# permon/permon

Measured on AMD Instinct MI355X. Metric: QPS iterations/sec + CSR SpMV GB/s (% HBM roofline), higher is better.
Workload: dtype f64; 1 GPU; configs[2]: 3-D elasticity TFETI contact, 2x2x2 subdomains of 43^3 Q1 elements (N=2044416 dof, n_lambda=102268), SMALXE+MPGP on the dual QP, F = B K^+ B' with K^+ explicit (dense local dual operators, storage class_orbit)

## Files before the change

### include/permon_hip.h

```cpp
#ifndef PERMON_HIP_H
#define PERMON_HIP_H

#include <stddef.h>
#include <stdint.h>

#ifdef __cplusplus
extern "C" {
#endif

#define PMH_SUCCESS 0
#define PMH_ERR_HIP 1
#define PMH_ERR_ARG 2
#define PMH_ERR_STATE 3
#define PMH_ERR_SUP 4
#define PMH_ERR_NODEVICE 5
#define PMH_ERR_COMM 6
const char *pmh_last_error(void);

#define PMH_CONVERGED_ITERATING 0
#define PMH_CONVERGED_RTOL 2
#define PMH_CONVERGED_ATOL 3
#define PMH_CONVERGED_ITS 4
#define PMH_CONVERGED_HAPPY_BREAKDOWN 7
#define PMH_DIVERGED_ITS (-3)
// ... 589 lines not shown
  double        astol, afeas, alpha, acg_host, pAp_host;
  double        ttol, divtol_rhs, gamma2;
  double        ring[48];
  double        scal_dev[64], scal_pinned[64];
  int           emit;
  int           spec;
  int           setp;
  int           finalize;
  int           use_ctl;
  int           nb;
  int           ring_cap, max_it;
  int           ctl[4];
} pmh_mpgp_phase_test;
enum { PMH_PHASE_SPLIT = 0, PMH_PHASE_STEP, PMH_PHASE_DIR, PMH_PHASE_PROP_DIR, PMH_PHASE_EXPANSION, PMH_PHASE_P1_DOTS, PMH_PHASE_THREE_NORMS, PMH_PHASE_OBJ };
int pmh_vec_test_finalize(pmh_ctx ctx, int K, int nblocks, const double *rows_host, const int *ops, const int *slots, int halt, int *post_inc, double *scal_dev, double *scal_pinned);
int pmh_mpgp_test_host_sum_row(const double *row, int nb, int op, double *out);
int pmh_mpgp_test_block_sum(pmh_ctx ctx, int nb, const double *row_host, double *out_host);
int pmh_mpgp_test_block_partials(pmh_ctx ctx, int n, const double *a, const double *b, const double *c, double *dev_host, double *pinned_host);
int pmh_mpgp_test_phase(pmh_ctx ctx, int phase, int n, pmh_mpgp_phase_test *t);
int pmh_mpgp_test_set_gradient_valid(pmh_mpgp s, const double *g);
int pmh_mpgp_test_spec_words(pmh_mpgp s, int words[5]);
int pmh_op_test_create_staged(pmh_csr gather, pmh_csr middle, pmh_csr scatter, pmh_op *op);
int pmh_op_penalized_test_chain_info(pmh_op op, long long info[10]);
int pmh_op_penalized_test_chain_read(pmh_op op, int what, int cap, double *host, int *len);
int pmh_op_penalized_test_norm_target(pmh_op op, double *Gu, int slot, const double *u, int *ready);
int pmh_op_penalized_test_mult_epi2(pmh_op op, int kind, int same_input, int in_slot, const double *x, const double *b, const double *g, const double *xx, const double *lb,
                                    const double *ub, double astol, double *y, double *gf, double *p, double *partials_dev_host, double *partials_pinned_host, int *nblocks,
                                    int *replayed);
int pmh_op_penalized_test_form(pmh_op op, int *form);
int pmh_op_penalized_test_aux_normG(pmh_op op, int armed, const double *u, double *Gu, int slot, const double *x, double *y, double scal[2], int *served);
// ... 17 lines not shown
```

### permon_amd/_lib.py

```python
import ctypes as C
import os

_HERE = os.path.dirname(os.path.abspath(__file__))
LIB_PATH = os.path.join(_HERE, "libpermonhip.so")

c_double_p = C.POINTER(C.c_double)
c_int_p = C.POINTER(C.c_int)
vp = C.c_void_p


class PermonHipError(RuntimeError):
    pass


class MpgpOpts(C.Structure):
    _fields_ = [
        ("rtol", C.c_double), ("atol", C.c_double), ("divtol", C.c_double), ("max_it", C.c_int),
        ("alpha_user", C.c_double), ("alpha_direct", C.c_int), ("gamma", C.c_double),
        ("maxeig", C.c_double), ("maxeig_tol", C.c_double), ("maxeig_iter", C.c_int),
        ("bchop_tol", C.c_double), ("astol", C.c_double),
        ("exptype", C.c_int), ("explengthtype", C.c_int),
        ("resetalpha", C.c_int), ("fallback", C.c_int), ("fallback2", C.c_int),
        ("monitor", C.c_int), ("unfused", C.c_int), ("distributed", C.c_int),
    ]
# ... 370 lines not shown
    "pmh_mg_create_sa": [vp, vp, C.c_int, vp, C.c_int, vp, vp, vp, C.c_int, vp, C.c_int, vp, C.c_int, C.c_double, C.c_int, C.c_int, C.POINTER(vp)],
    "pmh_mg_timing_enable": [vp, C.c_int],
    "pmh_mg_timing_get": [vp, C.POINTER(C.c_int), C.POINTER(C.c_double), C.POINTER(C.c_double)],
    "pmh_matinv_enable_bsr3": [vp],
    "pmh_matinv_bsr3_replicas": [vp, c_int_p],
    "pmh_mv_test_spmv": [vp, C.c_int, vp, vp, C.c_int, C.POINTER(C.c_float)],
    "pmh_mv_test_create": [vp, C.c_int, C.c_int, C.c_int, C.POINTER(vp)],
    "pmh_mv_test_info": [vp, C.POINTER(C.c_longlong), c_double_p],
    "pmh_mv_test_mult_epi": [vp, C.c_int, vp, vp, vp, vp, vp, vp, vp, C.c_double, C.c_double, C.c_double, C.c_int],
    "pmh_mv_test_destroy": [vp],
    "pmh_csr_kernel_info": [vp, c_int_p, C.POINTER(C.c_ulonglong)],
    "pmh_csr_test_mult_epi": [vp, C.c_int, vp, vp, vp, vp, vp, vp, C.c_int, vp, c_double_p],
    "pmh_op_penalized_test_mult_epi": [vp, C.c_int, C.c_int, vp, vp, vp, C.c_double, vp, vp, vp, C.c_int, vp, vp, c_int_p, c_int_p],
    "pmh_op_penalized_test_emit": [vp, C.c_int, vp],
    "pmh_vec_test_finalize": [vp, C.c_int, C.c_int, vp, vp, vp, C.c_int, vp, vp, vp],
    "pmh_mpgp_test_host_sum_row": [vp, C.c_int, C.c_int, c_double_p],
    "pmh_mpgp_test_block_sum": [vp, C.c_int, vp, vp],
    "pmh_mpgp_test_block_partials": [vp, C.c_int, vp, vp, vp, vp, vp],
    "pmh_mpgp_test_phase": [vp, C.c_int, C.c_int, C.POINTER(MpgpPhaseTest)],
    "pmh_mpgp_test_set_gradient_valid": [vp, vp],
    "pmh_mpgp_test_spec_words": [vp, c_int_p],
    "pmh_op_test_create_staged": [vp, vp, vp, C.POINTER(vp)],
    "pmh_op_penalized_test_chain_info": [vp, C.POINTER(C.c_longlong)],
    "pmh_op_penalized_test_chain_read": [vp, C.c_int, C.c_int, vp, c_int_p],
    "pmh_op_penalized_test_norm_target": [vp, vp, C.c_int, vp, c_int_p],
    "pmh_op_penalized_test_mult_epi2": [vp, C.c_int, C.c_int, C.c_int, vp, vp, vp, vp, vp, vp, C.c_double, vp, vp, vp, vp, vp, c_int_p, c_int_p],
    "pmh_op_penalized_test_form": [vp, c_int_p],
    "pmh_op_penalized_test_aux_normG": [vp, C.c_int, vp, vp, C.c_int, vp, vp, c_double_p, c_int_p],
    "pmh_bsr3_test_create": [vp, C.c_int, C.c_int, C.c_int, C.POINTER(vp)],
    "pmh_bsr3_test_info": [vp, C.POINTER(C.c_longlong), c_double_p],
# ... 106 lines not shown
```

### permon_amd/csrc/ctx.hip

```cpp
#include <sched.h>

#include <algorithm>
#include <thread>

#include "pmh_internal.h"

static thread_local char g_err[1024] = "";

int pmh_set_error(int code, const char *fmt, ...)
{
  va_list ap;
  va_start(ap, fmt);
  vsnprintf(g_err, sizeof(g_err), fmt, ap);
  va_end(ap);
  return code;
}

extern "C" const char *pmh_last_error(void) { return g_err; }

pmh_knobs_s &pmh_knobs()
{
  static pmh_knobs_s k = [] {
    pmh_knobs_s v;
    v.chain = getenv("PMH_NO_CHAIN") ? 0 : 1;
    v.chain_replay = getenv("PMH_NO_CHAIN_REPLAY") ? 0 : 1;
    v.svm_pairing = getenv("PMH_SVM_NO_PAIRING") ? 0 : 1;
    v.gt_fusion = getenv("PMH_NO_GT_FUSION") ? 0 : 1;
    v.multi_rhs = getenv("PMH_NO_MULTI_RHS") ? 0 : 1;
    v.kplus_mv = getenv("PMH_NO_KPLUS_MV") ? 0 : 1;
    v.smalxe_prefetch = getenv("PMH_SMALXE_NO_PREFETCH") ? 0 : 1;
    v.mg_d0_fusion = getenv("PMH_MG_NO_D0_FUSION") ? 0 : 1;
    v.vec_epi = getenv("PMH_NO_VEC_EPI") ? 0 : 1;
    v.mpgp_spec = getenv("PMH_MPGP_NO_SPEC") ? 0 : 1;
    v.orbit_adapted = getenv("PMH_NO_ORBIT_ADAPTED") ? 0 : 1;
    int         nt = 0;
    const char *e  = getenv("PMH_HOST_THREADS");
    if (!e) e = getenv("OMP_NUM_THREADS");
    if (e) nt = atoi(e);
    if (nt <= 0) {
      cpu_set_t set;
      CPU_ZERO(&set);
      nt = (sched_getaffinity(0, sizeof(set), &set) == 0) ? CPU_COUNT(&set) : (int)std::thread::hardware_concurrency();
      nt = std::min(16, nt);
    }
    v.host_threads = std::max(1, std::min(64, nt));
// ... 4 lines not shown
static int *knob_by_name(const char *name)
{
  if (!name) return nullptr;
  if (!strcmp(name, "chain")) return &pmh_knobs().chain;
  if (!strcmp(name, "chain_applies")) return &pmh_knobs().chain_applies;
  if (!strcmp(name, "chain_launches")) return &pmh_knobs().chain_launches;
  if (!strcmp(name, "chain_replay")) return &pmh_knobs().chain_replay;
  if (!strcmp(name, "chain_replays")) return &pmh_knobs().chain_replays;
  if (!strcmp(name, "chain_replays_redone")) return &pmh_knobs().chain_replays_redone;
  if (!strcmp(name, "host_threads")) return &pmh_knobs().host_threads;
  if (!strcmp(name, "svm_pairing")) return &pmh_knobs().svm_pairing;
  if (!strcmp(name, "gt_fusion")) return &pmh_knobs().gt_fusion;
  if (!strcmp(name, "multi_rhs")) return &pmh_knobs().multi_rhs;
  if (!strcmp(name, "kplus_mv")) return &pmh_knobs().kplus_mv;
  if (!strcmp(name, "smalxe_prefetch")) return &pmh_knobs().smalxe_prefetch;
  if (!strcmp(name, "mg_d0_fusion")) return &pmh_knobs().mg_d0_fusion;
  if (!strcmp(name, "mpgp_spec")) return &pmh_knobs().mpgp_spec;
  if (!strcmp(name, "vec_epi")) return &pmh_knobs().vec_epi;
  if (!strcmp(name, "orbit_adapted")) return &pmh_knobs().orbit_adapted;
  if (!strcmp(name, "orbit_adapted_classes")) return &pmh_knobs().orbit_adapted_classes;
  if (!strcmp(name, "orbit_adapted_fallbacks")) return &pmh_knobs().orbit_adapted_fallbacks;
  if (!strcmp(name, "orbit_adapted_spoil")) return &pmh_knobs().orbit_adapted_spoil;
  return nullptr;
}
extern "C" int pmh_set_knob(const char *name, int value)
{
  int *k = knob_by_name(name);
  if (!k) return pmh_set_error(PMH_ERR_ARG, "pmh_set_knob: unknown switch '%s'", name ? name : "(null)");
  *k = value;
  return PMH_SUCCESS;
// ... 67 lines not shown
  hipDeviceProp_t prop;
  PMH_HIP(hipGetDeviceProperties(&prop, c->device));
  snprintf(buf, len, "%s (%s, %d CUs)", prop.name, prop.gcnArchName, prop.multiProcessorCount);
  return PMH_SUCCESS;
}

extern "C" int pmh_mem_info(pmh_ctx c, size_t *free_bytes, size_t *total_bytes)
{
  PMH_ARG(c && free_bytes && total_bytes);
  PMH_HIP(hipSetDevice(c->device));
  PMH_HIP(hipStreamSynchronize(c->stream));
  PMH_HIP(hipMemGetInfo(free_bytes, total_bytes));
  return PMH_SUCCESS;
}

static inline hipError_t ctx_wait(pmh_ctx c) { return hipStreamSynchronize(c->stream); }

extern "C" int pmh_sync(pmh_ctx c)
{
  PMH_ARG(c);
  PMH_HIP(ctx_wait(c));
  return PMH_SUCCESS;
}

extern "C" void *pmh_stream(pmh_ctx c) { return c ? (void *)c->stream : nullptr; }

extern "C" int pmh_malloc(pmh_ctx c, size_t bytes, void **dptr)
{
  PMH_ARG(c && dptr);
  PMH_HIP(hipSetDevice(c->device));
  PMH_HIP(hipMalloc(dptr, bytes ? bytes : 8));
// ... 225 lines not shown
```

### permon_amd/csrc/dualchain.h

```cpp
#pragma once
#include "pmh_internal.h"

struct pmh_dualchain_s;
typedef pmh_dualchain_s *pmh_dualchain;

int  pmh_dc_create(pmh_qppf pf, pmh_op F, pmh_dualchain *out);
void pmh_dc_destroy(pmh_dualchain dc);
int  pmh_dc_apply(pmh_dualchain dc, const double *x, double *y, double rho, const pmh_vec_epi *epi);
int  pmh_dc_emit_begin(pmh_dualchain dc, const double *x, const double *p, pmh_emit_args *ea);
void pmh_dc_invalidate(pmh_dualchain dc, bool keep_applied = false);
int  pmh_dc_replay(pmh_dualchain dc, const double *x, double *y, double rho, const pmh_vec_epi *epi, int *replayed);
int  pmh_dc_test_emit(pmh_dualchain dc, const double *x);
int  pmh_dc_test_direction_sums(pmh_dualchain dc, int cap, double *host, int *nseg);
int  pmh_dc_set_norm_target(pmh_dualchain dc, double *Gu, int slot);
bool pmh_dc_norm_ready(pmh_dualchain dc, const double *u);
int  pmh_dc_last_launches(pmh_dualchain dc);
int  pmh_dc_test_info(pmh_dualchain dc, long long info[10]);
int  pmh_dc_test_read(pmh_dualchain dc, int what, int cap, double *host, int *len);
```

### permon_amd/csrc/dualchain.hip

```cpp
#include <algorithm>
#include <cmath>
#include <type_traits>

#include "dualchain.h"
#include "emit_inline.h"
#include "box_inline.h"
#include "reduce.h"

struct pmh_dualchain_s {
  pmh_ctx  ctx;
  pmh_qppf pf;
  pmh_op   F;
  int      n, m, nwg, nseg, W;
  pmh_csr  gather = nullptr, scatter = nullptr;
  double  *mid_in = nullptr;
  const double *mid_out = nullptr;
  int     *d_seg = nullptr, *d_lrow = nullptr;
  double        *d_ev = nullptr;
  unsigned char *d_ec = nullptr;
  pmh_csr  list_for = nullptr;
  unsigned long long list_uid = 0, sc_uid = 0;
  double  *zeroed   = nullptr;
  int      nlist = 0, *d_reci = nullptr;
  double  *d_recd = nullptr;
  pmh_csr  sc_for = nullptr;
  int     *d_sc2 = nullptr;
  double  *d_sv2 = nullptr;
  unsigned char *d_scnt = nullptr;
  double  *part[3] = {nullptr, nullptr, nullptr};
  double  *c_cur   = nullptr;
  double  *w       = nullptr;
  double  *normGu    = nullptr;
  int      norm_slot = -1;
  const double *x_emitted = nullptr;
  bool     norm_done = false;
  const double *norm_ptr = nullptr;
  int      launches = 0;
  const double      *kept_x     = nullptr;
  unsigned long long kept_epoch = 0;
};


__global__ __launch_bounds__(PMH_EMIT_TILE) void k_dc_emit(int n, const double *__restrict__ x, pmh_emit_args ea)
{
  pmh_emit_regs R;
  pmh_emit_prefetch(ea, R);
  const int r = blockIdx.x * PMH_EMIT_TILE + threadIdx.x;
  pmh_emit_tail(ea, R, r < n ? x[r] : 0.0, 0.0);
}

template <int NU>
// ... 449 lines not shown
}

static void dc_launch_emit(pmh_dualchain dc, const double *x, double *part)
{
  hipLaunchKernelGGL(k_dc_emit, dim3((unsigned)dc->nwg), dim3(PMH_EMIT_TILE), 0, dc->ctx->stream, dc->n, x, dc_emit_args(dc, part, nullptr));
}

int pmh_dc_emit_begin(pmh_dualchain dc, const double *x, const double *p, pmh_emit_args *ea)
{
  *ea = dc_emit_args(dc, x ? dc->part[0] : nullptr, p ? dc->part[1] : nullptr);
  if ((x && x == dc->kept_x) || (p && p == dc->kept_x)) dc->kept_x = nullptr;
  if (x) dc->x_emitted = x, dc->norm_done = false, dc->norm_ptr = nullptr;
  return PMH_SUCCESS;
}

void pmh_dc_invalidate(pmh_dualchain dc, bool keep_applied)
{
  dc->x_emitted = nullptr, dc->norm_ptr = nullptr, dc->norm_done = false;
  if (!keep_applied) dc->kept_x = nullptr;
}

int pmh_dc_set_norm_target(pmh_dualchain dc, double *Gu, int slot)
{
  PMH_ARG(dc && Gu && slot >= 0 && slot < PMH_NSCAL);
  dc->normGu = Gu, dc->norm_slot = slot, dc->norm_ptr = nullptr, dc->norm_done = false;
  return PMH_SUCCESS;
}

bool pmh_dc_norm_ready(pmh_dualchain dc, const double *u)
{
  if (!dc || !dc->normGu) return false;
  if (dc->norm_ptr == u) return true;
  if (dc->x_emitted == u && !dc->norm_done) {
// ... 34 lines not shown
  });
  dc->launches++;
  PMH_HIP(hipGetLastError());
  return PMH_SUCCESS;
}

int pmh_dc_apply(pmh_dualchain dc, const double *x, double *y, double rho, const pmh_vec_epi *epi)
{
  pmh_ctx     ctx = dc->ctx;
  hipStream_t st  = ctx->stream;
  const int   n = dc->n;
  const dim3  vgrid((unsigned)dc->nwg), eblk(PMH_EMIT_TILE);
  const int   kind = epi ? epi->kind : 0;
  dc->launches     = 0;
  dc->kept_x       = nullptr;
  const pmh_emit_tab tab = dc_tab(dc);
  int slot = (epi && epi->in_slot > 0) ? epi->in_slot - 1 : -1;
  if (slot < 0) {
    slot = (kind == PMH_VEPI_GRAD_SPLIT) ? 0 : (kind == PMH_VEPI_P1 ? 1 : 2);
    if (slot == 0) dc->x_emitted = x, dc->norm_done = false, dc->norm_ptr = nullptr;
    dc_launch_emit(dc, x, dc->part[slot]);
    dc->launches++;
  }
  PMH_CHK(dc->F->stages(&dc->gather, &dc->mid_in, &dc->scatter, &dc->mid_out));
  const pmh_csr Bg = dc->gather, Bs = dc->scatter;
  if (Bg->ncols != n || Bs->nrows != n) return pmh_set_error(PMH_ERR_STATE, "pmh_dc_apply: the operator's stages changed their dual dimension");
  PMH_CHK(dc_prepare_stages(dc));
  {
    dc_norm_args na;
    memset(&na, 0, sizeof(na));
// ... 25 lines not shown
int pmh_dc_replay(pmh_dualchain dc, const double *x, double *y, double rho, const pmh_vec_epi *epi, int *replayed)
{
  const int kind = epi ? epi->kind : 0;
  if (replayed) *replayed = 0;
  bool      ok   = pmh_knobs().chain_replay && x && dc->kept_x == x && dc->kept_epoch == dc->ctx->free_epoch && (kind == 0 || kind == PMH_VEPI_GRAD_SPLIT);
  if (ok) {
    pmh_csr       g = nullptr, sc = nullptr;
    double       *mi = nullptr;
    const double *mo = nullptr;
    PMH_CHK(dc->F->stages(&g, &mi, &sc, &mo));
    ok = g && sc && g == dc->list_for && g->uid == dc->list_uid && mi == dc->zeroed && sc == dc->sc_for && sc->uid == dc->sc_uid && mo == dc->mid_out;
  }
  if (!ok) return pmh_dc_apply(dc, x, y, rho, epi);
  dc->launches = 0;
  if (kind == PMH_VEPI_GRAD_SPLIT && !(epi->in_slot > 0)) {
    dc->x_emitted = x, dc->norm_done = false, dc->norm_ptr = nullptr;
    dc_launch_emit(dc, x, dc->part[0]);
    dc->launches++;
  }
  PMH_CHK(dc_last_stage(dc, x, y, rho, epi));
  if (replayed) *replayed = 1;
  pmh_knobs().chain_applies++, pmh_knobs().chain_replays++, pmh_knobs().chain_launches += dc->launches;
  return PMH_SUCCESS;
}

int pmh_dc_test_emit(pmh_dualchain dc, const double *x)
{
  pmh_emit_args ea;
  PMH_CHK(pmh_dc_emit_begin(dc, x, nullptr, &ea));
  dc_launch_emit(dc, x, ea.o[0].part);
  PMH_HIP(hipGetLastError());
  return PMH_SUCCESS;
}
int pmh_dc_test_direction_sums(pmh_dualchain dc, int cap, double *host, int *nseg)
// ... 81 lines not shown
```

### permon_amd/csrc/pmh_internal.h

```cpp
#pragma once
#include <hip/hip_runtime.h>
#include <rccl/rccl.h>

#include <cstdarg>
#include <cstdio>
#include <cstdlib>
#include <cstring>
#include <vector>

#include "permon_hip.h"

#define PMH_BLOCK 256
#define PMH_MAX_VEC_BLOCKS 2048
#define PMH_MAX_RED 8
#define PMH_NSCAL 64

int pmh_set_error(int code, const char *fmt, ...);

struct pmh_knobs_s {
  int chain;
  int chain_applies = 0, chain_launches = 0;
  int chain_replay = 1, chain_replays = 0, chain_replays_redone = 0;
  int gt_fusion = 1;
  int smalxe_prefetch = 1;
  int vec_epi = 1;
  int orbit_adapted = 1, orbit_adapted_classes = 0, orbit_adapted_fallbacks = 0, orbit_adapted_spoil = 0;
  int mpgp_spec = 1;
  int mg_d0_fusion = 1;
  int kplus_mv = 1;
  int multi_rhs = 1;
  int svm_pairing = 1;
  int host_threads = 1;
};
pmh_knobs_s &pmh_knobs();
inline int   pmh_host_threads() { return pmh_knobs().host_threads > 1 ? pmh_knobs().host_threads : 1; }

#define PMH_HIP(call) \
  do { \
    hipError_t e_ = (call); \
// ... 17 lines not shown
struct pmh_ctx_s {
  int         device;
  int         num_cus;
  hipStream_t stream;
  hipEvent_t  ev0, ev1;
  double     *d_partials;
  int         partials_cap;
  double     *d_scal;
  double     *h_scal;
  double     *h_partials;
  ncclComm_t comm;
  int        rank, size, force_comm;
  double    *d_commbuf;
  int        dist_scalars;
  unsigned long long free_epoch = 0;
  pmh_comm_host_fn hook      = nullptr;
  void            *hook_user = nullptr;
  double          *h_stage   = nullptr;
  size_t           stage_cap = 0;
  hipEvent_t *comm_ev      = nullptr;
  int         comm_ev_cap = 0, comm_ev_used = 0;
  double      comm_ev_bytes = 0.0;
};
static inline bool pmh_comm_on(pmh_ctx c) { return (c->comm || c->hook) && (c->size > 1 || c->force_comm); }
int pmh_comm_allreduce_scalars(pmh_ctx c, double *dscal, int K, const int *ops );
int pmh_comm_sum_host(pmh_ctx c, double *h, int k);

enum { PMH_SPMV_ELL = 0, PMH_SPMV_STREAM = 1, PMH_SPMV_MEDIUM = 2, PMH_SPMV_VECTOR = 3, PMH_SPMV_LONG = 4 };
struct pmh_csr_s {
  pmh_ctx   ctx;
// ... 107 lines not shown
  const double *row = nullptr;
  double        row_aat = 0.0;
  double       *or_part = nullptr, *or_s = nullptr;
};

int pmh_onerow_dot(pmh_qppf pf, const double *v, double coef, double *out);
int pmh_onerow_scaled_row(pmh_qppf pf, const double *s, double coef, const double *v , double *y);

enum { PMH_RED_SUM = 0, PMH_RED_MIN = 1 };
int pmh_finalize_partials(pmh_ctx ctx, const double *partials, int ld, int nblocks, int K, const int *ops, int scal_base, const int *halt = nullptr, int *post_inc = nullptr);
int pmh_finalize_partials_slots(pmh_ctx ctx, const double *partials, int ld, int nblocks, int K, const int *ops, const int *slots);
int pmh_vec_grid(int n);

int pmh_qpc_box_project_flag(pmh_ctx ctx, int n, const double *x, const double *lb, const double *ub, double *Px, int slot);
int pmh_k_dot_partials(pmh_ctx ctx, int n, const double *x, const double *y, int slot);
int pmh_qppf_apply_G_norm2(pmh_qppf pf, const double *v, double *Gv, int slot);
int pmh_mpgp_set_pre_test_hook(pmh_mpgp s, int (*f)(void *), void *user);
int pmh_mpgp_set_convergence_margin(pmh_mpgp s, double margin);
int pmh_mpgp_set_gradient_valid(pmh_mpgp s, int valid, double **g);
int pmh_mpgp_x_applied(pmh_mpgp s);
int pmh_mpgp_set_first_operand_applied(pmh_mpgp s, int on);
int pmh_mpgp_set_pre_p1_hook(pmh_mpgp s, int (*f)(void *), void *user);
int pmh_op_penalized_arm_aux_normG(pmh_op op, const double *u, double *Gu, int slot);
enum { PMH_PEN_FOLD = 0, PMH_PEN_CHAIN = 1, PMH_PEN_ONE_LAUNCH = 2, PMH_PEN_TEN_LAUNCH = 3, PMH_PEN_DENSE_INVERSE = 4, PMH_PEN_PLAIN = 5 };
int pmh_op_penalized_take_aux_done(pmh_op op);
int pmh_op_penalized_set_normG_target(pmh_op op, double *Gu, int slot);
int pmh_op_penalized_normG_ready(pmh_op op, const double *u);
int pmh_op_penalized_chain_launches(pmh_op op);
#define PMH_SLOT_NORMBU2 48
#define PMH_SLOT_PROJ_CHANGED 52
// ... 42 lines not shown
```

### permon_amd/csrc/qppf.hip

```cpp
#include <chrono>

#include "pmh_internal.h"
#include "reduce.h"
#include "box_inline.h"
#include "dualchain.h"
#include "svm_internal.h"


__global__ __launch_bounds__(PMH_BLOCK) void k_dense_gemv(int m, const double *__restrict__ M, const double *__restrict__ x, double *__restrict__ y)
{
  const int row = blockIdx.x * (PMH_BLOCK / 64) + (threadIdx.x >> 6), lane = threadIdx.x & 63;
  if (row >= m) return;
  double s = 0.0;
  for (int j = lane; j < m; j += 64) s += M[(size_t)row * m + j] * x[j];
  s = pmh_wave_sum(s);
  if (lane == 0) y[row] = s;
}

typedef double v4f64 __attribute__((ext_vector_type(4)));
#define GGT_KCHUNK 8192

__global__ __launch_bounds__(PMH_BLOCK) void k_densify_gt(int m, int Mp, const int *__restrict__ rowptr, const int *__restrict__ col, const double *__restrict__ val, double *__restrict__ Gt)
{
  const int row = blockIdx.x;
// ... 640 lines not shown
  int fold_apply(const double *x, double *y, const pmh_vec_epi *e)
  {
    const double *au = aux_u;
    sv->sigma_fold   = rho * sv_c * sv_c;
    sv->aux_done     = 0;
    if (au) sv->aux_u = au, sv->aux_Gu = aux_Gu, sv->aux_slot = aux_slot, sv->aux_c = sv_c;
    const int rc   = e ? sv->mult_epi(x, y, *e) : sv->mult(x, y);
    sv->sigma_fold = 0.0, sv->aux_u = nullptr;
    if (rc != PMH_EPI_UNSUPPORTED) aux_u = nullptr;
    if (sv->aux_done) aux_done = 1, sv->aux_done = 0;
    return rc;
  }
  int  emit_begin(const double *x, const double *p, pmh_emit_args *ea) override { return chain() ? pmh_dc_emit_begin(dc, x, p, ea) : PMH_EPI_UNSUPPORTED; }
  void emit_invalidate(bool keep_applied = false) override
  {
    if (dc) pmh_dc_invalidate(dc, keep_applied);
  }
  bool one_launch() { return projected() && gt_fusable(pf) && q_fused_dense(pf); }
  int form()
  {
    if (fold()) return PMH_PEN_FOLD;
    if (chain()) return PMH_PEN_CHAIN;
    if (projected()) {
      if (gt_fusable(pf)) return q_fused_dense(pf) ? PMH_PEN_ONE_LAUNCH : PMH_PEN_TEN_LAUNCH;
      if (gt_fusable_dense_inverse(pf)) return PMH_PEN_DENSE_INVERSE;
    }
    return PMH_PEN_PLAIN;
  }
  int mult_fused_dense(const double *x, double *y, const pmh_vec_epi *epi)
  {
    ProjectedOp *pa = static_cast<ProjectedOp *>(A);
    const double *au = aux_u;
// ... 135 lines not shown
}

int pmh_op_penalized_set_normG_target(pmh_op op, double *Gu, int slot)
{
  PenalizedOp *o = dynamic_cast<PenalizedOp *>(op);
  PMH_ARG(o && Gu && slot >= 0 && slot < PMH_NSCAL);
  o->norm_Gu = Gu, o->norm_slot = slot;
  if (o->dc) PMH_CHK(pmh_dc_set_norm_target(o->dc, Gu, slot));
  return PMH_SUCCESS;
}
int pmh_op_penalized_normG_ready(pmh_op op, const double *u)
{
  PenalizedOp *o = dynamic_cast<PenalizedOp *>(op);
  return (o && o->dc && pmh_dc_norm_ready(o->dc, u)) ? 1 : 0;
}
int pmh_op_penalized_chain_launches(pmh_op op)
{
  PenalizedOp *o = dynamic_cast<PenalizedOp *>(op);
  return (o && o->dc) ? pmh_dc_last_launches(o->dc) : -1;
}

extern "C" int pmh_op_penalized_test_emit(pmh_op op, int what, const double *x)
{
  PenalizedOp *o = dynamic_cast<PenalizedOp *>(op);
  PMH_ARG(o && (what == 0 || (what == 1 && x)));
  if (!o->chain()) return pmh_set_error(PMH_ERR_SUP, "pmh_op_penalized_test_emit: the operator does not run on the dual-space chain");
  if (what == 0) {
    o->emit_invalidate();
    return PMH_SUCCESS;
  }
  return pmh_dc_test_emit(o->dc, x);
}

extern "C" int pmh_op_penalized_test_mult_epi(pmh_op op, int kind, int same_input, const double *x, const double *b, const double *lb, double astol, double *y, double *gf, double *p, int cap,
                                              double *partials_host, double *psums_host, int *nblocks, int *nseg)
{
  PenalizedOp *o = dynamic_cast<PenalizedOp *>(op);
  PMH_ARG(o && x && y && (kind == 0 || kind == PMH_VEPI_GRAD_SPLIT));
  if (!o->chain()) return pmh_set_error(PMH_ERR_SUP, "pmh_op_penalized_test_mult_epi: the operator does not run on the dual-space chain");
  pmh_ctx ctx = o->ctx;
  if (kind == 0) {
    PMH_CHK(same_input ? o->mult_same_input(x, y) : o->mult(x, y));
    return pmh_sync(ctx);
// ... 152 lines not shown
```

### permon_amd/csrc/smalxe.hip

```cpp
#include <cmath>

#include "pmh_internal.h"

struct pmh_smalxe_s {
  pmh_ctx         ctx;
  pmh_op          A;
  const double   *b;
  double         *u;
  const double   *lb, *ub;
  pmh_qppf        pf;
  pmh_smalxe_opts o;
  int             n;
  double M1, M1_initial, eta, maxeig;
  int    M1_updates, M1_hits, eta_hits, rho_updates;
  int    state, inner_iter_accu;
  double normBu, normBu_old, enorm;
  double rnorm;
  int    iteration, reason;
  pmh_op   A_inner;
  pmh_mpgp inner;
  double  *Btmu, *b_inner, *BtBu, *Bu, *xwork;
  int      normBu_prefetched;
  double gtol, ttol_outer, norm_rhs_outer, MNormBu;
  double outer_norm_rhs, outer_ttol, outer_norm_rhs_div;
  int    outer_cvg_setup;
  double inner_atol;
  int    inner_reason, inner_max_it;
  double inner_rnorm;
  int    BtBu_valid, inner_it_now;
  double lag_normBu0;
  int    lag_II, lag_J, lag_neval, lag_niter;
  int reuse;
  int normBu_final_valid;
  int Btmu_given;
};

extern "C" int pmh_smalxe_default_opts(pmh_smalxe_opts *o)
{
  PMH_ARG(o);
  memset(o, 0, sizeof(*o));
  o->rtol               = 1e-5;
  o->atol               = 1e-50;
  o->divtol             = 1e4;
  o->max_it             = 100;
  o->M1_user            = 1e2;
  o->M1_direct          = 0;
  o->M1_update          = 2.0;
  o->rtol_E             = 1e-0;
  o->rho_user           = 1.1;
// ... 103 lines not shown
  if (s->lag_II == s->lag_J) {
    s->lag_II = 0;
    if (s->lag_J < s->o.lag_end) s->lag_J += s->o.lag_step;
  }
  *normBu = normBu_approx;
  *enorm  = *normBu / s->o.rtol_E;
  return PMH_SUCCESS;
}

static int update_normBu(pmh_smalxe s, const double *u, double *normBu, double *enorm)
{
  if (!s->o.be_implicit || s->pf->m == 0) return update_normBu_std(s, u, normBu, enorm);
  return s->o.lag_enabled ? update_normBu_lag(s, u, normBu, enorm) : update_normBu_on(s, u, normBu, enorm);
}

static int outer_converged(pmh_smalxe s, int *reason)
{
  if (!s->outer_cvg_setup) {
    PMH_CHK(pmh_vec_norm2(s->ctx, s->n, s->b, &s->outer_norm_rhs));
    s->outer_ttol         = fmax(s->o.rtol * s->outer_norm_rhs, s->o.atol);
    s->outer_norm_rhs_div = s->outer_norm_rhs;
    s->outer_cvg_setup    = 1;
  }
  *reason = PMH_CONVERGED_ITERATING;
  if (s->iteration > s->o.max_it) {
    *reason = PMH_DIVERGED_ITS;
    return PMH_SUCCESS;
  }
  if (std::isnan(s->rnorm) || std::isinf(s->rnorm)) *reason = PMH_DIVERGED_NANORINF;
  else if (s->rnorm <= s->outer_ttol) *reason = (s->rnorm < s->o.atol) ? PMH_CONVERGED_ATOL : PMH_CONVERGED_RTOL;
  else if (s->rnorm >= s->o.divtol * s->outer_norm_rhs_div) *reason = PMH_DIVERGED_DTOL;
  return PMH_SUCCESS;
}

static int inner_converged(void *user, int i, double gnorm, int *reason)
{
  pmh_smalxe s = (pmh_smalxe)user;
  *reason      = PMH_CONVERGED_ITERATING;
// ... 50 lines not shown
  PMH_ARG(ctx && A && b && u && pf && o && out);
  PMH_ARG(pf->n == A->n);
  pmh_smalxe s = new pmh_smalxe_s();
  memset((void *)s, 0, sizeof(*s));
  s->ctx = ctx, s->A = A, s->b = b, s->u = u, s->lb = lb, s->ub = ub, s->pf = pf, s->o = *o, s->n = A->n;
  s->state  = 1;
  s->normBu = s->normBu_old = s->enorm = NAN;
  s->reuse      = 0;
  const int n = s->n;
  PMH_CHK(pmh_malloc(ctx, sizeof(double) * (size_t)n, (void **)&s->BtBu));
  PMH_CHK(pmh_malloc(ctx, sizeof(double) * (size_t)n, (void **)&s->Btmu));
  PMH_CHK(pmh_malloc(ctx, sizeof(double) * (size_t)n, (void **)&s->b_inner));
  PMH_CHK(pmh_malloc(ctx, sizeof(double) * (size_t)n, (void **)&s->xwork));
  PMH_CHK(pmh_malloc(ctx, sizeof(double) * (size_t)(pf->m ? pf->m : 1), (void **)&s->Bu));
  PMH_CHK(pmh_memset(ctx, s->Btmu, 0, sizeof(double) * (size_t)n));

  s->eta = s->o.eta_user;
  if (!s->o.eta_direct) {
    double normb;
    PMH_CHK(pmh_vec_norm2(ctx, n, b, &normb));
    s->eta *= normb;
  }
  s->maxeig     = s->o.maxeig;
  s->M1_initial = s->o.M1_user;
  if (!s->o.M1_direct) {
    if (s->maxeig == PMH_DECIDE) PMH_CHK(pmh_op_max_eigenvalue(A, s->o.maxeig_tol, s->o.maxeig_iter, &s->maxeig, nullptr));
    s->M1_initial *= s->maxeig;
  }
  double rho;
  if (!s->o.rho_direct) {
    if (s->maxeig == PMH_DECIDE) PMH_CHK(pmh_op_max_eigenvalue(A, s->o.maxeig_tol, s->o.maxeig_iter, &s->maxeig, nullptr));
    rho = s->o.rho_user * s->maxeig;
  } else {
    rho = s->o.rho_user;
  }
  PMH_CHK(pmh_op_create_penalized(A, pf, rho, &s->A_inner));
  PMH_CHK(pmh_vec_copy(ctx, n, b, s->b_inner));

  pmh_mpgp_opts io       = s->o.inner;
  s->inner_max_it        = io.max_it;
  const double maxeig_in = fmax(rho, s->maxeig);
  int          inject    = s->o.inject_maxeig_set ? s->o.inject_maxeig : pf->orthonormal;
  if (inject) io.maxeig = maxeig_in;
  PMH_CHK(pmh_mpgp_create(ctx, s->A_inner, s->b_inner, u, lb, ub, &io, &s->inner));
  PMH_CHK(pmh_mpgp_set_convergence_test(s->inner, inner_converged, s));
  PMH_CHK(pmh_mpgp_set_pre_test_hook(s->inner, prefetch_normBu, s));
  PMH_CHK(pmh_mpgp_set_pre_p1_hook(s->inner, arm_normBu, s));
  if (!s->o.be_implicit && pf->m > 0 && pf->implicit_orth && pf->m <= 64) PMH_CHK(pmh_op_penalized_set_normG_target(s->A_inner, s->Bu, PMH_SLOT_NORMBU2));
  *out = s;
  return PMH_SUCCESS;
}
// ... 3 lines not shown
  PMH_ARG(s);
  s->reuse = on ? 1 : 0;
  return PMH_SUCCESS;
}

extern "C" int pmh_smalxe_destroy(pmh_smalxe s)
{
  if (!s) return PMH_SUCCESS;
  pmh_mpgp_destroy(s->inner);
  pmh_op_destroy(s->A_inner);
  pmh_free(s->ctx, s->BtBu);
  pmh_free(s->ctx, s->Btmu);
  pmh_free(s->ctx, s->b_inner);
  pmh_free(s->ctx, s->xwork);
  pmh_free(s->ctx, s->Bu);
  delete s;
  return PMH_SUCCESS;
}

static int objective(pmh_smalxe s, double *f, bool after_inner)
{
  if (after_inner && pmh_mpgp_x_applied(s->inner)) PMH_CHK(s->A_inner->mult_same_input(s->u, s->xwork));
  else PMH_CHK(s->A_inner->mult(s->u, s->xwork));
  PMH_CHK(pmh_vec_aypx(s->ctx, s->n, s->xwork, -0.5, s->b_inner));
  double dot;
  PMH_CHK(pmh_vec_dot(s->ctx, s->n, s->u, s->xwork, &dot));
  *f = -dot;
  return PMH_SUCCESS;
}

static int smalxe_update(pmh_smalxe s, double Lag_old, double Lag, double rho)
{
  double t    = 0.5 * rho * s->normBu * s->normBu;
  double t2   = Lag - (Lag_old + t);
  int    flag = (t2 < s->o.update_threshold);
  if (flag && s->o.M1_update != 1.0) {
    if (s->inner_reason == PMH_CONVERGED_ATOL) {
      s->M1 = s->M1 / s->o.M1_update;
      s->M1_updates++;
    }
  }
// ... 33 lines not shown
{
  PMH_ARG(s);
  pmh_ctx ctx = s->ctx;
  const int n = s->n, maxits = s->o.max_it;
  double  Lag, Lag_old, rho;
  int     i;

  s->M1 = s->M1_initial;
  PMH_CHK(pmh_op_penalized_get_penalty(s->A_inner, &rho));
  const int given = s->Btmu_given;
  s->Btmu_given   = 0;
  if (!given) PMH_CHK(pmh_memset(ctx, s->Btmu, 0, sizeof(double) * (size_t)n));
  s->BtBu_valid = 0;
  if (given) PMH_CHK(pmh_qpc_box_project(ctx, n, s->u, s->lb, s->ub, s->u));
  if (s->o.knoll && !given) PMH_CHK(pmh_qppf_apply_P(s->pf, s->b, s->u));
  PMH_CHK(objective(s, &Lag_old, false));
  bool u_applied = given != 0;
  PMH_CHK(update_normBu(s, s->u, &s->normBu_old, &s->enorm));
  s->iteration       = 0;
  s->inner_iter_accu = 0;
  s->reason          = PMH_CONVERGED_ITERATING;
  PMH_CHK(pmh_mpgp_reset_statistics(s->inner));
  if (given) {
    PMH_CHK(given_pair_converged(s));
    if (s->reason) return PMH_SUCCESS;
  }

  for (i = 0; i < maxits; i++) {
    if (!(given && i == 0)) {
      if (!s->BtBu_valid) PMH_CHK(pmh_qppf_apply_GtG(s->pf, s->u, s->BtBu));
      s->BtBu_valid = 1;
      PMH_CHK(pmh_vec_axpy(ctx, n, s->Btmu, rho, s->BtBu));
    }
    if (s->reason) break;
    PMH_CHK(pmh_vec_waxpy(ctx, n, s->b_inner, -1.0, s->Btmu, s->b));
    if (i == 0) PMH_CHK(pmh_vec_norm2(ctx, n, s->b, &s->norm_rhs_outer));
    s->gtol       = s->o.rtol * s->norm_rhs_outer;
    s->ttol_outer = fmax(s->o.rtol * s->norm_rhs_outer, s->o.atol);
    PMH_CHK(pmh_vec_norm2(ctx, n, s->b_inner, &s->outer_norm_rhs_div));
    PMH_CHK(pmh_mpgp_set_tolerances(s->inner, s->o.inner.rtol, s->o.inner.atol, s->o.divtol, s->inner_max_it));
    s->normBu_prefetched = 0;
    s->normBu_final_valid = 0;
    if (s->reuse && i > 0) {
      double  rho_now, *g = nullptr;
      PMH_CHK(pmh_op_penalized_get_penalty(s->A_inner, &rho_now));
      PMH_CHK(pmh_mpgp_set_gradient_valid(s->inner, 1, &g));
      if (g) PMH_CHK(pmh_vec_axpy(ctx, n, g, rho_now, s->BtBu));
    }
    PMH_CHK(pmh_mpgp_set_first_operand_applied(s->inner, u_applied && !s->reuse));
    u_applied = false;
    PMH_CHK(pmh_mpgp_solve(s->inner));
    pmh_mpgp_stats st;
    PMH_CHK(pmh_mpgp_get_stats(s->inner, &st));
    s->inner_reason = st.reason;
    s->inner_rnorm  = st.rnorm;
    s->inner_iter_accu += st.iteration;
    s->inner_it_now = st.iteration;
    s->BtBu_valid   = 0;
    s->iteration = i + 1;
    if (!(s->normBu_final_valid && !s->o.be_implicit && !s->o.lag_enabled)) PMH_CHK(update_normBu(s, s->u, &s->normBu, &s->enorm));
    PMH_CHK(pmh_op_penalized_get_penalty(s->A_inner, &rho));
    if (s->reuse) {
      double *g = nullptr, dot;
      PMH_CHK(pmh_mpgp_set_gradient_valid(s->inner, 0, &g));
      PMH_ARG(g);
      PMH_CHK(pmh_vec_waxpy(ctx, n, s->xwork, -1.0, g, s->b_inner));
      PMH_CHK(pmh_vec_dot(ctx, n, s->u, s->xwork, &dot));
      Lag = -0.5 * dot;
    } else {
      PMH_CHK(objective(s, &Lag, true));
      u_applied = true;
    }
    PMH_CHK(smalxe_update(s, Lag_old, Lag, rho));
    Lag_old       = Lag;
    s->normBu_old = s->normBu;
  }
  if (i == maxits && !s->reason) s->reason = PMH_DIVERGED_ITS;
  return PMH_SUCCESS;
}

extern "C" int pmh_smalxe_set_initial_multiplier(pmh_smalxe s, const double *Btmu0_dev)
{
// ... 145 lines not shown
```

### permon_amd/csrc/vec.hip

```cpp
#include <algorithm>
#include <cstdlib>

#include "pmh_internal.h"
#include "reduce.h"
#include "box_inline.h"

int pmh_vec_grid(int n)
{
  const int epb = 256;
  long long b = ((long long)n + epb - 1) / epb;
  if (b < 1) b = 1;
  if (b > PMH_MAX_VEC_BLOCKS) b = PMH_MAX_VEC_BLOCKS;
  return (int)b;
}

#define GRID_STRIDE(i, n) for (long long i = (long long)blockIdx.x * PMH_BLOCK + threadIdx.x; i < (n); i += (long long)gridDim.x * PMH_BLOCK)

struct pmh_ops8 {
  int op[PMH_MAX_RED];
  int slot[PMH_MAX_RED];
};

#define PMH_FIN_THREADS 1024
__global__ __launch_bounds__(PMH_FIN_THREADS) void k_finalize(const double *__restrict__ partials, int ld, int nblocks, int K, pmh_ops8 ops, double *__restrict__ d_scal, double *__restrict__ h_scal, const int *__restrict__ halt, int *__restrict__ post_inc)
// ... 175 lines not shown
extern "C" int pmh_vec_dot(pmh_ctx ctx, int n, const double *x, const double *y, double *result_host)
{
  PMH_ARG(ctx && n >= 0 && result_host);
  PMH_CHK(pmh_k_dot_partials(ctx, n, x, y, 0));
  return pmh_host_scalar(ctx, 0, result_host);
}

extern "C" int pmh_vec_norm2(pmh_ctx ctx, int n, const double *x, double *result_host)
{
  double s;
  PMH_CHK(pmh_vec_dot(ctx, n, x, x, &s));
  *result_host = sqrt(s);
  return PMH_SUCCESS;
}

__global__ __launch_bounds__(PMH_BLOCK) void k_box_project(long long n, const double *x, const double *lb, const double *ub, double *Px)
{
  GRID_STRIDE(i, n)
  {
    double v = x[i];
    if (lb) {
      double l = lb[i];
      v        = (v > l) ? v : l;
      if (ub) {
        double u = ub[i];
        v        = (v < u) ? v : u;
      }
    } else if (ub) {
      double u = ub[i];
      v        = (v < u) ? v : u;
// ... 129 lines not shown
```

Before: 4801 QPS iterations/s.

## Fuse SMALXE outer-loop vector updates with reductions and defer rhs-norm sync

Merges the multiplier update, inner right-hand-side formation and its norm into one kernel that writes per-block partials to mapped host memory. The host sums them later, and only syncs if no other sync has happened since. The Lagrangian's waxpy and dot are likewise fused into one kernel with a host-side sum. The dual-chain operator can also keep a previously emitted stage across invalidation so the emit launch is not repeated. This cuts kernel launches, vector passes and host waits per outer iteration, at the cost of more state-tracking complexity and a host finalize that must match the device reduction order.

```diff
diff --git a/include/permon_hip.h b/include/permon_hip.h
--- a/include/permon_hip.h
+++ b/include/permon_hip.h
@@ -627,6 +627,8 @@
 } pmh_mpgp_phase_test;
 enum { PMH_PHASE_SPLIT = 0, PMH_PHASE_STEP, PMH_PHASE_DIR, PMH_PHASE_PROP_DIR, PMH_PHASE_EXPANSION, PMH_PHASE_P1_DOTS, PMH_PHASE_THREE_NORMS, PMH_PHASE_OBJ };
 int pmh_vec_test_finalize(pmh_ctx ctx, int K, int nblocks, const double *rows_host, const int *ops, const int *slots, int halt, int *post_inc, double *scal_dev, double *scal_pinned);
+int pmh_vec_test_mult_rhs(pmh_ctx ctx, int n, double *Btmu, double rho, const double *BtBu, const double *b, double *b_inner, double *row_host, int *nblocks, double *sum);
+int pmh_vec_test_waxpy_dot(pmh_ctx ctx, int n, double *w, double a, const double *x, const double *y, const double *u, double *row_host, int *nblocks, double *sum);
 int pmh_mpgp_test_host_sum_row(const double *row, int nb, int op, double *out);
 int pmh_mpgp_test_block_sum(pmh_ctx ctx, int nb, const double *row_host, double *out_host);
 int pmh_mpgp_test_block_partials(pmh_ctx ctx, int n, const double *a, const double *b, const double *c, double *dev_host, double *pinned_host);
diff --git a/permon_amd/_lib.py b/permon_amd/_lib.py
--- a/permon_amd/_lib.py
+++ b/permon_amd/_lib.py
@@ -408,6 +408,8 @@
     "pmh_op_penalized_test_mult_epi": [vp, C.c_int, C.c_int, vp, vp, vp, C.c_double, vp, vp, vp, C.c_int, vp, vp, c_int_p, c_int_p],
     "pmh_op_penalized_test_emit": [vp, C.c_int, vp],
     "pmh_vec_test_finalize": [vp, C.c_int, C.c_int, vp, vp, vp, C.c_int, vp, vp, vp],
+    "pmh_vec_test_mult_rhs": [vp, C.c_int, vp, C.c_double, vp, vp, vp, vp, c_int_p, c_double_p],
+    "pmh_vec_test_waxpy_dot": [vp, C.c_int, vp, C.c_double, vp, vp, vp, vp, c_int_p, c_double_p],
     "pmh_mpgp_test_host_sum_row": [vp, C.c_int, C.c_int, c_double_p],
     "pmh_mpgp_test_block_sum": [vp, C.c_int, vp, vp],
     "pmh_mpgp_test_block_partials": [vp, C.c_int, vp, vp, vp, vp, vp],
diff --git a/permon_amd/csrc/ctx.hip b/permon_amd/csrc/ctx.hip
--- a/permon_amd/csrc/ctx.hip
+++ b/permon_amd/csrc/ctx.hip
@@ -29,6 +29,7 @@
     v.multi_rhs = getenv("PMH_NO_MULTI_RHS") ? 0 : 1;
     v.kplus_mv = getenv("PMH_NO_KPLUS_MV") ? 0 : 1;
     v.smalxe_prefetch = getenv("PMH_SMALXE_NO_PREFETCH") ? 0 : 1;
+    v.smalxe_outer_fused = getenv("PMH_SMALXE_OUTER_UNFUSED") ? 0 : 1;
     v.mg_d0_fusion = getenv("PMH_MG_NO_D0_FUSION") ? 0 : 1;
     v.vec_epi = getenv("PMH_NO_VEC_EPI") ? 0 : 1;
     v.mpgp_spec = getenv("PMH_MPGP_NO_SPEC") ? 0 : 1;
@@ -63,6 +64,9 @@
   if (!strcmp(name, "multi_rhs")) return &pmh_knobs().multi_rhs;
   if (!strcmp(name, "kplus_mv")) return &pmh_knobs().kplus_mv;
   if (!strcmp(name, "smalxe_prefetch")) return &pmh_knobs().smalxe_prefetch;
+  if (!strcmp(name, "smalxe_outer_fused")) return &pmh_knobs().smalxe_outer_fused;
+  if (!strcmp(name, "chain_emits_kept")) return &pmh_knobs().chain_emits_kept;
+  if (!strcmp(name, "host_waits")) return &pmh_knobs().host_waits;
   if (!strcmp(name, "mg_d0_fusion")) return &pmh_knobs().mg_d0_fusion;
   if (!strcmp(name, "mpgp_spec")) return &pmh_knobs().mpgp_spec;
   if (!strcmp(name, "vec_epi")) return &pmh_knobs().vec_epi;
@@ -160,7 +164,11 @@
   return PMH_SUCCESS;
 }
 
-static inline hipError_t ctx_wait(pmh_ctx c) { return hipStreamSynchronize(c->stream); }
+static inline hipError_t ctx_wait(pmh_ctx c)
+{
+  c->waits++, pmh_knobs().host_waits++;
+  return hipStreamSynchronize(c->stream);
+}
 
 extern "C" int pmh_sync(pmh_ctx c)
 {
diff --git a/permon_amd/csrc/dualchain.h b/permon_amd/csrc/dualchain.h
--- a/permon_amd/csrc/dualchain.h
+++ b/permon_amd/csrc/dualchain.h
@@ -8,7 +8,7 @@
 void pmh_dc_destroy(pmh_dualchain dc);
 int  pmh_dc_apply(pmh_dualchain dc, const double *x, double *y, double rho, const pmh_vec_epi *epi);
 int  pmh_dc_emit_begin(pmh_dualchain dc, const double *x, const double *p, pmh_emit_args *ea);
-void pmh_dc_invalidate(pmh_dualchain dc, bool keep_applied = false);
+void pmh_dc_invalidate(pmh_dualchain dc, bool keep_applied = false, bool keep_emitted = false);
 int  pmh_dc_replay(pmh_dualchain dc, const double *x, double *y, double rho, const pmh_vec_epi *epi, int *replayed);
 int  pmh_dc_test_emit(pmh_dualchain dc, const double *x);
 int  pmh_dc_test_direction_sums(pmh_dualchain dc, int cap, double *host, int *nseg);
diff --git a/permon_amd/csrc/dualchain.hip b/permon_amd/csrc/dualchain.hip
--- a/permon_amd/csrc/dualchain.hip
+++ b/permon_amd/csrc/dualchain.hip
@@ -35,6 +35,7 @@
   const double *x_emitted = nullptr;
   bool     norm_done = false;
   const double *norm_ptr = nullptr;
+  bool     emitted_kept = false;
   int      launches = 0;
   const double      *kept_x     = nullptr;
   unsigned long long kept_epoch = 0;
@@ -514,9 +515,10 @@
   return PMH_SUCCESS;
 }
 
-void pmh_dc_invalidate(pmh_dualchain dc, bool keep_applied)
-{
-  dc->x_emitted = nullptr, dc->norm_ptr = nullptr, dc->norm_done = false;
+void pmh_dc_invalidate(pmh_dualchain dc, bool keep_applied, bool keep_emitted)
+{
+  dc->emitted_kept = keep_applied && keep_emitted && dc->kept_x && dc->x_emitted == dc->kept_x && dc->kept_epoch == dc->ctx->free_epoch;
+  if (!dc->emitted_kept) dc->x_emitted = nullptr, dc->norm_ptr = nullptr, dc->norm_done = false;
   if (!keep_applied) dc->kept_x = nullptr;
 }
 
@@ -581,6 +583,7 @@
   const int   kind = epi ? epi->kind : 0;
   dc->launches     = 0;
   dc->kept_x       = nullptr;
+  dc->emitted_kept = false;
   const pmh_emit_tab tab = dc_tab(dc);
   int slot = (epi && epi->in_slot > 0) ? epi->in_slot - 1 : -1;
   if (slot < 0) {
@@ -636,10 +639,15 @@
   if (!ok) return pmh_dc_apply(dc, x, y, rho, epi);
   dc->launches = 0;
   if (kind == PMH_VEPI_GRAD_SPLIT && !(epi->in_slot > 0)) {
-    dc->x_emitted = x, dc->norm_done = false, dc->norm_ptr = nullptr;
-    dc_launch_emit(dc, x, dc->part[0]);
-    dc->launches++;
-  }
+    if (dc->emitted_kept && dc->x_emitted == x) {
+      pmh_knobs().chain_emits_kept++;
+    } else {
+      dc->x_emitted = x, dc->norm_done = false, dc->norm_ptr = nullptr;
+      dc_launch_emit(dc, x, dc->part[0]);
+      dc->launches++;
+    }
+  }
+  dc->emitted_kept = false;
   PMH_CHK(dc_last_stage(dc, x, y, rho, epi));
   if (replayed) *replayed = 1;
   pmh_knobs().chain_applies++, pmh_knobs().chain_replays++, pmh_knobs().chain_launches += dc->launches;
diff --git a/permon_amd/csrc/pmh_internal.h b/permon_amd/csrc/pmh_internal.h
--- a/permon_amd/csrc/pmh_internal.h
+++ b/permon_amd/csrc/pmh_internal.h
@@ -23,6 +23,7 @@
   int chain_replay = 1, chain_replays = 0, chain_replays_redone = 0;
   int gt_fusion = 1;
   int smalxe_prefetch = 1;
+  int smalxe_outer_fused = 1, chain_emits_kept = 0, host_waits = 0;
   int vec_epi = 1;
   int orbit_adapted = 1, orbit_adapted_classes = 0, orbit_adapted_fallbacks = 0, orbit_adapted_spoil = 0;
   int mpgp_spec = 1;
@@ -70,6 +71,7 @@
   double    *d_commbuf;
   int        dist_scalars;
   unsigned long long free_epoch = 0;
+  unsigned long long waits = 0;
   pmh_comm_host_fn hook      = nullptr;
   void            *hook_user = nullptr;
   double          *h_stage   = nullptr;
@@ -207,6 +209,10 @@
 
 int pmh_qpc_box_project_flag(pmh_ctx ctx, int n, const double *x, const double *lb, const double *ub, double *Px, int slot);
 int pmh_k_dot_partials(pmh_ctx ctx, int n, const double *x, const double *y, int slot);
+int    pmh_vec_mult_rhs(pmh_ctx ctx, int n, double *Btmu, double rho, const double *BtBu, const double *b, double *b_inner, double *row, int *nb);
+int    pmh_vec_waxpy_dot(pmh_ctx ctx, int n, double *w, double a, const double *x, const double *y, const double *u, double *row, int *nb);
+double pmh_host_finalize_sum(const double *row, int nb);
+int pmh_op_penalized_set_keep_emitted(pmh_op op, int on);
 int pmh_qppf_apply_G_norm2(pmh_qppf pf, const double *v, double *Gv, int slot);
 int pmh_mpgp_set_pre_test_hook(pmh_mpgp s, int (*f)(void *), void *user);
 int pmh_mpgp_set_convergence_margin(pmh_mpgp s, double margin);
diff --git a/permon_amd/csrc/qppf.hip b/permon_amd/csrc/qppf.hip
--- a/permon_amd/csrc/qppf.hip
+++ b/permon_amd/csrc/qppf.hip
@@ -678,8 +678,9 @@
   int  emit_begin(const double *x, const double *p, pmh_emit_args *ea) override { return chain() ? pmh_dc_emit_begin(dc, x, p, ea) : PMH_EPI_UNSUPPORTED; }
   void emit_invalidate(bool keep_applied = false) override
   {
-    if (dc) pmh_dc_invalidate(dc, keep_applied);
-  }
+    if (dc) pmh_dc_invalidate(dc, keep_applied, keep_emitted != 0);
+  }
+  int keep_emitted = 0;
   bool one_launch() { return projected() && gt_fusable(pf) && q_fused_dense(pf); }
   int form()
   {
@@ -845,6 +846,13 @@
   PenalizedOp *o = dynamic_cast<PenalizedOp *>(op);
   return (o && o->dc && pmh_dc_norm_ready(o->dc, u)) ? 1 : 0;
 }
+int pmh_op_penalized_set_keep_emitted(pmh_op op, int on)
+{
+  PenalizedOp *o = dynamic_cast<PenalizedOp *>(op);
+  PMH_ARG(o);
+  o->keep_emitted = on ? 1 : 0;
+  return PMH_SUCCESS;
+}
 int pmh_op_penalized_chain_launches(pmh_op op)
 {
   PenalizedOp *o = dynamic_cast<PenalizedOp *>(op);
@@ -854,10 +862,17 @@
 extern "C" int pmh_op_penalized_test_emit(pmh_op op, int what, const double *x)
 {
   PenalizedOp *o = dynamic_cast<PenalizedOp *>(op);
-  PMH_ARG(o && (what == 0 || (what == 1 && x)));
+  PMH_ARG(o && (what == 0 || what == 2 || (what == 1 && x)));
   if (!o->chain()) return pmh_set_error(PMH_ERR_SUP, "pmh_op_penalized_test_emit: the operator does not run on the dual-space chain");
   if (what == 0) {
     o->emit_invalidate();
+    return PMH_SUCCESS;
+  }
+  if (what == 2) {
+    const int was   = o->keep_emitted;
+    o->keep_emitted = 1;
+    o->emit_invalidate(true);
+    o->keep_emitted = was;
     return PMH_SUCCESS;
   }
   return pmh_dc_test_emit(o->dc, x);
diff --git a/permon_amd/csrc/smalxe.hip b/permon_amd/csrc/smalxe.hip
--- a/permon_amd/csrc/smalxe.hip
+++ b/permon_amd/csrc/smalxe.hip
@@ -33,6 +33,11 @@
   int reuse;
   int normBu_final_valid;
   int Btmu_given;
+  int                outer_fused;
+  double            *h_outer;
+  int                rhs_pending;
+  int                rhs_nb;
+  unsigned long long rhs_waits;
 };
 
 extern "C" int pmh_smalxe_default_opts(pmh_smalxe_opts *o)
@@ -166,6 +171,15 @@
   return s->o.lag_enabled ? update_normBu_lag(s, u, normBu, enorm) : update_normBu_on(s, u, normBu, enorm);
 }
 
+static int settle_rhs_norm(pmh_smalxe s)
+{
+  if (!s->rhs_pending) return PMH_SUCCESS;
+  if (s->ctx->waits == s->rhs_waits) PMH_CHK(pmh_sync(s->ctx));
+  s->outer_norm_rhs_div = sqrt(pmh_host_finalize_sum(s->h_outer, s->rhs_nb));
+  s->rhs_pending        = 0;
+  return PMH_SUCCESS;
+}
+
 static int outer_converged(pmh_smalxe s, int *reason)
 {
   if (!s->outer_cvg_setup) {
@@ -174,6 +188,7 @@
     s->outer_norm_rhs_div = s->outer_norm_rhs;
     s->outer_cvg_setup    = 1;
   }
+  PMH_CHK(settle_rhs_norm(s));
   *reason = PMH_CONVERGED_ITERATING;
   if (s->iteration > s->o.max_it) {
     *reason = PMH_DIVERGED_ITS;
@@ -254,6 +269,8 @@
   PMH_CHK(pmh_malloc(ctx, sizeof(double) * (size_t)n, (void **)&s->xwork));
   PMH_CHK(pmh_malloc(ctx, sizeof(double) * (size_t)(pf->m ? pf->m : 1), (void **)&s->Bu));
   PMH_CHK(pmh_memset(ctx, s->Btmu, 0, sizeof(double) * (size_t)n));
+  s->outer_fused = pmh_knobs().smalxe_outer_fused && !s->o.inner.distributed;
+  if (s->outer_fused) PMH_HIP(hipHostMalloc((void **)&s->h_outer, sizeof(double) * 2 * PMH_MAX_VEC_BLOCKS, hipHostMallocMapped));
 
   s->eta = s->o.eta_user;
   if (!s->o.eta_direct) {
@@ -275,6 +292,7 @@
     rho = s->o.rho_user;
   }
   PMH_CHK(pmh_op_create_penalized(A, pf, rho, &s->A_inner));
+  PMH_CHK(pmh_op_penalized_set_keep_emitted(s->A_inner, s->outer_fused));
   PMH_CHK(pmh_vec_copy(ctx, n, b, s->b_inner));
 
   pmh_mpgp_opts io       = s->o.inner;
@@ -308,7 +326,18 @@
   pmh_free(s->ctx, s->b_inner);
   pmh_free(s->ctx, s->xwork);
   pmh_free(s->ctx, s->Bu);
+  if (s->h_outer) (void)hipHostFree(s->h_outer);
   delete s;
+  return PMH_SUCCESS;
+}
+
+static int lagrangian_dot(pmh_smalxe s, double a, const double *x, const double *y, double *dot)
+{
+  double *row = s->h_outer + PMH_MAX_VEC_BLOCKS;
+  int     nb;
+  PMH_CHK(pmh_vec_waxpy_dot(s->ctx, s->n, s->xwork, a, x, y, s->u, row, &nb));
+  PMH_CHK(pmh_sync(s->ctx));
+  *dot = pmh_host_finalize_sum(row, nb);
   return PMH_SUCCESS;
 }
 
@@ -316,9 +345,13 @@
 {
   if (after_inner && pmh_mpgp_x_applied(s->inner)) PMH_CHK(s->A_inner->mult_same_input(s->u, s->xwork));
   else PMH_CHK(s->A_inner->mult(s->u, s->xwork));
-  PMH_CHK(pmh_vec_aypx(s->ctx, s->n, s->xwork, -0.5, s->b_inner));
   double dot;
-  PMH_CHK(pmh_vec_dot(s->ctx, s->n, s->u, s->xwork, &dot));
+  if (s->outer_fused) {
+    PMH_CHK(lagrangian_dot(s, -0.5, s->xwork, s->b_inner, &dot));
+  } else {
+    PMH_CHK(pmh_vec_aypx(s->ctx, s->n, s->xwork, -0.5, s->b_inner));
+    PMH_CHK(pmh_vec_dot(s->ctx, s->n, s->u, s->xwork, &dot));
+  }
   *f = -dot;
   return PMH_SUCCESS;
 }
@@ -382,6 +415,7 @@
   s->BtBu_valid = 0;
   if (given) PMH_CHK(pmh_qpc_box_project(ctx, n, s->u, s->lb, s->ub, s->u));
   if (s->o.knoll && !given) PMH_CHK(pmh_qppf_apply_P(s->pf, s->b, s->u));
+  if (s->outer_fused) s->A_inner->emit_invalidate();
   PMH_CHK(objective(s, &Lag_old, false));
   bool u_applied = given != 0;
   PMH_CHK(update_normBu(s, s->u, &s->normBu_old, &s->enorm));
@@ -395,17 +429,26 @@
   }
 
   for (i = 0; i < maxits; i++) {
+    const bool fused = s->outer_fused && !(given && i == 0) && !s->reason;
     if (!(given && i == 0)) {
       if (!s->BtBu_valid) PMH_CHK(pmh_qppf_apply_GtG(s->pf, s->u, s->BtBu));
       s->BtBu_valid = 1;
-      PMH_CHK(pmh_vec_axpy(ctx, n, s->Btmu, rho, s->BtBu));
+      if (fused) {
+        PMH_CHK(pmh_vec_mult_rhs(ctx, n, s->Btmu, rho, s->BtBu, s->b, s->b_inner, s->h_outer, &s->rhs_nb));
+        s->rhs_pending = 1, s->rhs_waits = ctx->waits;
+      } else {
+        PMH_CHK(pmh_vec_axpy(ctx, n, s->Btmu, rho, s->BtBu));
+      }
     }
     if (s->reason) break;
-    PMH_CHK(pmh_vec_waxpy(ctx, n, s->b_inner, -1.0, s->Btmu, s->b));
+    if (!fused) PMH_CHK(pmh_vec_waxpy(ctx, n, s->b_inner, -1.0, s->Btmu, s->b));
     if (i == 0) PMH_CHK(pmh_vec_norm2(ctx, n, s->b, &s->norm_rhs_outer));
     s->gtol       = s->o.rtol * s->norm_rhs_outer;
     s->ttol_outer = fmax(s->o.rtol * s->norm_rhs_outer, s->o.atol);
-    PMH_CHK(pmh_vec_norm2(ctx, n, s->b_inner, &s->outer_norm_rhs_div));
+    if (!fused) {
+      s->rhs_pending = 0;
+      PMH_CHK(pmh_vec_norm2(ctx, n, s->b_inner, &s->outer_norm_rhs_div));
+    }
     PMH_CHK(pmh_mpgp_set_tolerances(s->inner, s->o.inner.rtol, s->o.inner.atol, s->o.divtol, s->inner_max_it));
     s->normBu_prefetched = 0;
     s->normBu_final_valid = 0;
@@ -432,8 +475,12 @@
       double *g = nullptr, dot;
       PMH_CHK(pmh_mpgp_set_gradient_valid(s->inner, 0, &g));
       PMH_ARG(g);
-      PMH_CHK(pmh_vec_waxpy(ctx, n, s->xwork, -1.0, g, s->b_inner));
-      PMH_CHK(pmh_vec_dot(ctx, n, s->u, s->xwork, &dot));
+      if (s->outer_fused) {
+        PMH_CHK(lagrangian_dot(s, -1.0, g, s->b_inner, &dot));
+      } else {
+        PMH_CHK(pmh_vec_waxpy(ctx, n, s->xwork, -1.0, g, s->b_inner));
+        PMH_CHK(pmh_vec_dot(ctx, n, s->u, s->xwork, &dot));
+      }
       Lag = -0.5 * dot;
     } else {
       PMH_CHK(objective(s, &Lag, true));
diff --git a/permon_amd/csrc/vec.hip b/permon_amd/csrc/vec.hip
--- a/permon_amd/csrc/vec.hip
+++ b/permon_amd/csrc/vec.hip
@@ -213,6 +213,93 @@
   return PMH_SUCCESS;
 }
 
+__global__ __launch_bounds__(PMH_BLOCK) void k_mult_rhs(long long n, double *__restrict__ Btmu, double rho, const double *__restrict__ BtBu, const double *__restrict__ b, double *__restrict__ b_inner,
+                                                        double *__restrict__ row)
+{
+  __shared__ double lds[PMH_BLOCK / 64];
+  double            s = 0.0;
+  GRID_STRIDE(i, n)
+  {
+    double m = Btmu[i];
+    m += rho * BtBu[i];
+    Btmu[i]        = m;
+    const double w = -1.0 * m + b[i];
+    b_inner[i]     = w;
+    s += w * w;
+  }
+  s = pmh_block_reduce<PMH_RED_SUM>(s, lds);
+  if (threadIdx.x == 0) row[blockIdx.x] = s;
+}
+__global__ __launch_bounds__(PMH_BLOCK) void k_waxpy_dot(long long n, double *w, double a, const double *x, const double *y, const double *__restrict__ u, double *__restrict__ row)
+{
+  __shared__ double lds[PMH_BLOCK / 64];
+  double            s = 0.0;
+  GRID_STRIDE(i, n)
+  {
+    const double v = a * x[i] + y[i];
+    w[i]           = v;
+    s += u[i] * v;
+  }
+  s = pmh_block_reduce<PMH_RED_SUM>(s, lds);
+  if (threadIdx.x == 0) row[blockIdx.x] = s;
+}
+
+int pmh_vec_mult_rhs(pmh_ctx ctx, int n, double *Btmu, double rho, const double *BtBu, const double *b, double *b_inner, double *row, int *nb)
+{
+  PMH_ARG(ctx && n >= 0 && row && nb);
+  *nb = n > 0 ? pmh_vec_grid(n) : 0;
+  LAUNCH_VEC(k_mult_rhs, n, Btmu, rho, BtBu, b, b_inner, row);
+  return PMH_SUCCESS;
+}
+int pmh_vec_waxpy_dot(pmh_ctx ctx, int n, double *w, double a, const double *x, const double *y, const double *u, double *row, int *nb)
+{
+  PMH_ARG(ctx && n >= 0 && row && nb);
+  *nb = n > 0 ? pmh_vec_grid(n) : 0;
+  LAUNCH_VEC(k_waxpy_dot, n, w, a, x, y, u, row);
+  return PMH_SUCCESS;
+}
+
+double pmh_host_finalize_sum(const double *row, int nb)
+{
+  double waves[PMH_FIN_THREADS / 64];
+  for (int w = 0; w < PMH_FIN_THREADS / 64; w++) {
+    double v[64];
+    for (int l = 0; l < 64; l++) {
+      v[l] = 0.0;
+      for (int i = 64 * w + l; i < nb; i += PMH_FIN_THREADS) v[l] = v[l] + row[i];
+    }
+    for (int o = 32; o > 0; o >>= 1)
+      for (int l = 0; l < o; l++) v[l] = v[l] + v[l + o];
+    waves[w] = v[0];
+  }
+  double r = waves[0];
+  for (int w = 1; w < PMH_FIN_THREADS / 64; w++) r = r + waves[w];
+  return r;
+}
+
+static int test_outer_row(pmh_ctx ctx, int which, int n, double *v0, double a, const double *v1, const double *v2, double *v3, const double *v4, double *row_host, int *nblocks, double *sum)
+{
+  PMH_ARG(ctx && n >= 0 && row_host && nblocks && sum);
+  double *row = nullptr;
+  PMH_HIP(hipHostMalloc((void **)&row, sizeof(double) * PMH_MAX_VEC_BLOCKS, hipHostMallocMapped));
+  int rc = which == 0 ? pmh_vec_mult_rhs(ctx, n, v0, a, v1, v2, v3, row, nblocks) : pmh_vec_waxpy_dot(ctx, n, v0, a, v1, v2, v4, row, nblocks);
+  if (!rc) rc = pmh_sync(ctx);
+  if (!rc) {
+    memcpy(row_host, row, sizeof(double) * (size_t)*nblocks);
+    *sum = pmh_host_finalize_sum(row, *nblocks);
+  }
+  (void)hipHostFree(row);
+  return rc;
+}
+extern "C" int pmh_vec_test_mult_rhs(pmh_ctx ctx, int n, double *Btmu, double rho, const double *BtBu, const double *b, double *b_inner, double *row_host, int *nblocks, double *sum)
+{
+  return test_outer_row(ctx, 0, n, Btmu, rho, BtBu, b, b_inner, nullptr, row_host, nblocks, sum);
+}
+extern "C" int pmh_vec_test_waxpy_dot(pmh_ctx ctx, int n, double *w, double a, const double *x, const double *y, const double *u, double *row_host, int *nblocks, double *sum)
+{
+  return test_outer_row(ctx, 1, n, w, a, x, y, nullptr, u, row_host, nblocks, sum);
+}
+
 __global__ __launch_bounds__(PMH_BLOCK) void k_box_project(long long n, const double *x, const double *lb, const double *ub, double *Px)
 {
   GRID_STRIDE(i, n)
```

Result: no change. 4706 QPS iterations/s (median of 2 runs) (-2.0%).
